# nianticlabs/panoptic-forecasting

Hardware: AMD Instinct MI355X
Metric: forecast frames/sec @1024x2048, 3-in->dt=3 bg (higher is better)
Workload: dtype f32 as 2 fp16 terms/operand, 3 MFMA products, f32 accumulate (strict f32: fp32_only); 1 GPU; configs[1] bg short-term forecast 3-in dt=3 @1024x2048: 3 warp/splats + HarDNet-70 + upsample/argmax; resident_frames_per_gpu=128, streams=4, sub_batch=32, launch=hipGraph replay, sub-batches staggered, weights=random-init, calibrated (tests/golden/calib_seed1234.json), world=1, device=AMD Radeon Graphics, backend=single process

## Files before the change

panoptic-forecasting_amd/csrc/conv_dma.hip:

```cpp
#include <cstring>

#include "conv_epilogue.h"
#include "pf_prof.h"

#ifndef PF_PROBE
#define PF_PROBE 0
#endif
#if PF_PROBE
#define DPROBE(i) do { if (threadIdx.x == 0 && blockIdx.x == 5 && blockIdx.y == 0 && blockIdx.z == 0 && a.probe) a.probe[i] = wall_clock64(); } while (0)
#else
#define DPROBE(i) do { } while (0)
#endif

namespace pf {

typedef float f32x4 __attribute__((ext_vector_type(4)));

template <int KS, int STRIDE, int WM, int WK, int NT, int RV = 0>
struct DmaCfg {
    static constexpr int KC = dma_kc_ct(KS, STRIDE);
    static constexpr int MP = 4;
    static constexpr int TWT = WM == 1 ? 1 : 2;
    static constexpr int TW = 16 * TWT;
    static constexpr int TH = WM * MP / TWT;
// ... 306 lines not shown
            const int ox = tileX * C::TW + (mt % C::TWT) * 16 + (lane_e >> 4) * 4;
            if (oy >= a.Hout || ox >= a.Wout) continue;
            const bool pool_top = a.pool && ((m / C::TWT) & 1) == 0 && m + C::TWT < C::MP && oy + 1 < a.Hout;
            if (a.pool && !pool_top) continue;
            ResTaps t0, t1;
            if (has_res) {
                t0 = res_taps(a, rw, oy, ox);
                if (pool_top) t1 = res_taps(a, rw, oy + 1, ox);
            }
#pragma unroll
            for (int n = 0; n < NT; ++n) {
                const int co = (tile0 + n) * 16 + (lane_e & 15);
                if (epi_skip(a, co)) continue;
                const lds_float *chan = res_lds + (n * 16 + (lane_e & 15)) * rw.cs;
                const f32x4 top = epi_finish(a, b, co, oy, ox, acc[m][n], biasv[n], has_res, chan, &t0);
                if (!a.pool) epi_store(a, b, co, oy, ox, top, vmax);
                else epi_store_pooled(a, b, co, oy, ox, top, epi_finish(a, b, co, oy + 1, ox, acc[(m + C::TWT) % C::MP][n], biasv[n], has_res, chan, &t1), vmax);
                __builtin_amdgcn_sched_barrier(0);
            }
            DPROBE(5 + m);
        }
    }
    range_commit(a.status, a.range_slot, vmax);
    DPROBE(4);
#endif
}

template <int KS, int STRIDE, int WM, int WK, int NT, int EPI, int RV = 0, int KACC = 0>
static int launch_dma_epi(const ConvArgs &a0, int B, hipStream_t s) {
    if constexpr (KACC == 0 && EPI == 0 && RV == 0 && KS == 3) {
        if (a0.kacc) return launch_dma_epi<KS, STRIDE, WM, WK, NT, EPI, RV, 1>(a0, B, s);
// ... 126 lines not shown
```

panoptic-forecasting_amd/csrc/conv_epilogue.h:

```cpp
#pragma once
#include "conv_mfma.h"

namespace pf {

typedef float epi_f32x4 __attribute__((ext_vector_type(4)));
typedef float epi_f32x2 __attribute__((ext_vector_type(2)));
typedef __attribute__((address_space(3))) float lds_float;

__device__ __forceinline__ void lin_coord(int o, float scale, int in_size, int &i0, int &i1, float &l0, float &l1) {
#pragma clang fp contract(off)
    const float r = scale * (float)o;
    i0 = min((int)r, in_size - 1);
    i1 = i0 + (i0 < in_size - 1 ? 1 : 0);
    l1 = fminf(fmaxf(r - (float)i0, 0.f), 1.f);
    l0 = 1.f - l1;
}


__host__ __device__ inline int res_extent(int n_out, float scale) { return (int)(scale * (float)(n_out - 1)) + 3; }
__host__ __device__ inline int res_chan_stride(int rows, int cols) { return (rows * cols) | 1; }

struct ResWin {
    int sy0, sx0, rows, cols, cs;
};

__device__ __forceinline__ ResWin res_window(const ConvArgs &a, int oy0, int th, int ox0, int tw) {
    ResWin w;
    const int oy1 = min(oy0 + th, a.Hout) - 1, ox1 = min(ox0 + tw, a.Wout) - 1;
    w.sy0 = min((int)(a.res_sh * (float)oy0), a.Hres - 1);
    w.sx0 = min((int)(a.res_sw * (float)ox0), a.Wres - 1);
    w.rows = min((int)(a.res_sh * (float)oy1), a.Hres - 1) + 2 - w.sy0;
    w.cols = min((int)(a.res_sw * (float)ox1), a.Wres - 1) + 2 - w.sx0;
    w.cs = res_chan_stride(w.rows, w.cols);
    return w;
}

__device__ __forceinline__ void res_stage(const ConvArgs &a, const ResWin &w, int b, int co0, int nco, lds_float *lds,
                                          int tid, int nthr) {
    const int per = w.rows * w.cols;
    const size_t plane = (size_t)a.Hres * a.Wres;
    const float *base = a.res + ((size_t)b * a.res_ctotal + a.res_choff + co0) * plane;
    for (int e0 = 0; e0 < per; e0 += 64) {
        const int e = e0 + (tid & 63);
        const int r = e / w.cols, x = e - r * w.cols;
        const size_t off = (size_t)min(w.sy0 + r, a.Hres - 1) * a.Wres + min(w.sx0 + x, a.Wres - 1);
#pragma unroll 4
        for (int c = tid >> 6; c < nco; c += nthr >> 6)
            if (e < per && co0 + c < a.Cout) lds[c * w.cs + e] = base[(size_t)c * plane + off];
    }
}

struct ResTaps {
    int o0[4], o1[4];
    float lx1[4], hy1;
};
__device__ __forceinline__ ResTaps res_taps(const ConvArgs &a, const ResWin &w, int oy, int ox) {
    ResTaps t;
    int y0, y1;
    float hy0;
    lin_coord(oy, a.res_sh, a.Hres, y0, y1, hy0, t.hy1);
#pragma unroll
    for (int r = 0; r < 4; ++r) {
        int x0, x1;
// ... 95 lines not shown
            *reinterpret_cast<epi_h2 *>(p + 4) = epi_h2{hi[0], hi[1]};
            *reinterpret_cast<epi_h2 *>(p + 4 + d.term) = epi_h2{mid[0], mid[1]};
        }
        if (ok1) {
            *reinterpret_cast<epi_h2 *>(p + d.hw * 8) = epi_h2{hi[2], hi[3]};
            *reinterpret_cast<epi_h2 *>(p + d.hw * 8 + d.term) = epi_h2{mid[2], mid[3]};
        }
    }
}
__device__ __forceinline__ epi_f32x4 s4_finish(epi_f32x4 acc, float scale, const epi_f32x4 &bias4, float relu_lo) {
#pragma unroll
    for (int r = 0; r < 4; ++r) acc[r] = fmaxf(acc[r] * scale + bias4[r], relu_lo);
    return acc;
}

__device__ __forceinline__ void epi_store(const ConvArgs &a, int b, int co, int oy, int ox, epi_f32x4 v, float &vmax) {
    vmax = range_acc(vmax, v[0], v[1], v[2], v[3]);
    if (a.dst_fmt) {
        if (co >= a.Cout) v = epi_f32x4{0.f, 0.f, 0.f, 0.f};
        const epi_f32x4 c = quad_transpose(v);
        const int k = threadIdx.x & 3;
        if (ox + k < a.Wout)
            s4_store_px(s4_dst(a, b, (size_t)a.Hout * a.Wout), co & ~3, (size_t)oy * a.Wout + ox + k, c);
        return;
    }
    float *p = a.dst + ((size_t)b * a.dst_ctotal + a.dst_choff + co) * ((size_t)a.Hout * a.Wout) + (size_t)oy * a.Wout + ox;
    if ((a.Wout & 3) == 0 && ox + 3 < a.Wout) {
        if (a.accum) v += *reinterpret_cast<const epi_f32x4 *>(p);
        *reinterpret_cast<epi_f32x4 *>(p) = v;
    } else {
#pragma unroll
        for (int r = 0; r < 4; ++r)
            if (ox + r < a.Wout) p[r] = a.accum ? p[r] + v[r] : v[r];
    }
}

__device__ __forceinline__ void epi_store_pooled(const ConvArgs &a, int b, int co, int oy, int ox, epi_f32x4 top, epi_f32x4 bot, float &vmax) {
    const int Hp = a.Hout >> 1, Wp = a.Wout >> 1, py = oy >> 1, px = ox >> 1;
// ... 23 lines not shown
```

panoptic-forecasting_amd/csrc/conv_mfma.h:

```cpp
#pragma once
#include "conv_pack.h"
#include "pf_blob.h"
#include "pf_common.h"

namespace pf {

struct ConvArgs {
    const float *src[kConvMaxSrc];
    int src_ctotal[kConvMaxSrc];
    int src_choff[kConvMaxSrc];
    int src_cstart[kConvMaxSrc + 1];
    int src_chunk0[kConvMaxSrc + 1];
    int n_src;
    const float *wpk;
    const float *bias;
    float *dst;
    int dst_ctotal, dst_choff;
    int Cin, Cout, Hin, Win, Hout, Wout;
    int tilesX, tilesY, nchunks, relu;
    const float *zero_page;
    int ntiles;
    int no_bias;
    int pool;
    const float *res;
    int res_ctotal, res_choff, Hres, Wres;
    float res_sh, res_sw;
    int res_lds_off;
    int res_rows, res_cols;
    unsigned res_magic_cs, res_magic_cols;
    const float *wrem;
    int rem;
    int src_begin, src_end;
    int chunk_begin, chunk_end;
    long long *probe;
    unsigned *status;
    unsigned *range_slot;
    int kacc;
    int accum;
    float acc_scale;
    int dst_fmt;
    int dst_c4;
    int dst_limit;
    int src_fmt;
    int src_c4[kConvMaxSrc];
    int src_g0[kConvMaxSrc];
    int src_gn[kConvMaxSrc];
    int src_ent0[kConvMaxSrc + 1];
    float *share;
    int share_off;
    int share_cout;
    float share_scale;
    const float *fold_w;
    const float *fold_bias;
    float fold_scale;
    const float *fold_src;
    int fold_c4, fold_g0, fold_gn;
    float *tail_dst;
    int fold_cout, tail_ctotal, tail_choff;
    float *down_dst;
    int down_c4, down_choff, down_limit;
    int down_fmt, down_ctotal;
    unsigned *down_status, *down_slot;
};

typedef _Float16 split_t;
typedef split_t split_x2 __attribute__((ext_vector_type(2)));
typedef split_t split_x4 __attribute__((ext_vector_type(4)));
typedef split_t split_x8 __attribute__((ext_vector_type(8)));
constexpr float kSplitMaxAbs = 65504.f;
__device__ __forceinline__ void split_terms2(float x0, float x1, split_x2 &hi, split_x2 &mid) {
#if defined(__HIP_DEVICE_COMPILE__)
    typedef float f32x2 __attribute__((ext_vector_type(2)));
    hi = __builtin_convertvector(f32x2{x0, x1}, split_x2);
// ... 220 lines not shown
```

panoptic-forecasting_amd/csrc/conv_s4.hip:

```cpp
#include <cstring>

#include "conv_s4.h"
#include "pf_prof.h"

#ifndef PF_PROBE
#define PF_PROBE 0
#endif
#if PF_PROBE
#define S4_PROBE(i) do { if (threadIdx.x == 0 && blockIdx.x == gridDim.x / 2 && blockIdx.y == 0 && blockIdx.z == gridDim.z / 2 && a.probe && (i) < 60) a.probe[i] = clock64(); } while (0)
#else
#define S4_PROBE(i) do { } while (0)
#endif

[[maybe_unused]] constexpr int kS4IssueFirst = 1, kS4IssueStep = 2;

namespace pf {

template <int NT, int TW_, int TH_ = 8, int KS_ = 1>
struct S4Cfg {
    static constexpr int TW = TW_, TH = TH_, MTR = TW / 16, MP = 2 * MTR;
    static constexpr int KS = KS_;
    static constexpr int NW = TH / 2, NTHR = 64 * NW;
    static constexpr int IW = TW + 4, IH = TH + 2;
    static constexpr int ROWP = IW / 2, PIECES = IH * ROWP;
// ... 126 lines not shown
    if (a.share_cout != a.Cout) return fail(PF_EINVAL, "conv_s4 add: stored sums of %d channels for %d", a.share_cout, a.Cout);
    PF_S4_SHARE(S4_ADD)
}
#undef PF_S4_SHARE
static int check_fold(const ConvArgs &a, const char *who, int max_cout, int ntiles = 2) {
    if (int rc = check_s4_form(a, who, false)) return rc;
    if (a.ntiles != ntiles) return fail(PF_EUNSUPPORTED, "%s: %d cout tiles, the form is built for %d", who, a.ntiles, ntiles);
    if (!a.fold_w || !a.fold_bias || a.fold_cout < 1 || a.fold_cout > max_cout || a.fold_gn < 0 || a.fold_gn > 8 || (a.fold_gn && !a.fold_src) ||
        (reinterpret_cast<uintptr_t>(a.fold_w) & 15) != 0 || (reinterpret_cast<uintptr_t>(a.fold_bias) & 15) != 0 || a.fold_g0 < 0 ||
        a.fold_g0 + a.fold_gn > a.fold_c4)
        return fail(PF_EINVAL, "%s: second conv of %d couts over %d groups", who, a.fold_cout, a.fold_gn);
    return PF_OK;
}
int launch_conv_s4_tail(const ConvArgs &a, int B, hipStream_t s) {
    if (int rc = check_fold(a, "conv_s4 tail", 16)) return rc;
    if (!a.tail_dst || a.tail_choff < 0 || a.tail_choff + a.fold_cout > a.tail_ctotal)
        return fail(PF_EINVAL, "conv_s4 tail: second conv of %d couts over %d groups", a.fold_cout, a.fold_gn);
    return launch_s4_form<S4_TAIL, 2>(a, B, s);
}
int launch_conv_s4_down(const ConvArgs &a, int B, hipStream_t s) {
    const bool wide = a.ntiles == 3;
    if (int rc = check_fold(a, "conv_s4 down", 16 * (wide ? kWideTiles : kDownTiles), wide ? 3 : 2)) return rc;
    if (a.Hout < 2 || a.Wout < 2) return fail(PF_EUNSUPPORTED, "conv_s4 down: nothing to pool at %d x %d", a.Hout, a.Wout);
    const bool packed_ok = (a.down_choff & 1) == 0 && a.down_limit >= a.down_choff + a.fold_cout && a.down_limit <= 4 * a.down_c4 &&
                           a.down_limit <= (a.down_choff + a.fold_cout + 3) / 4 * 4;
    if (!a.down_dst || a.down_choff < 0 || (a.down_fmt ? !packed_ok : a.down_choff + a.fold_cout > a.down_ctotal))
        return fail(PF_EINVAL, "conv_s4 down: pooled destination of %d channels from %d (limit %d) in %d groups", a.fold_cout, a.down_choff, a.down_limit, a.down_c4);
    return wide ? launch_s4_form<S4_DOWN, 3>(a, B, s) : launch_s4_form<S4_DOWN, 2>(a, B, s);
}
int launch_conv_s4_lo(const ConvArgs &a, int B, hipStream_t s) {
    if (int rc = check_fold(a, "conv_s4 lo", 16 * kLoTiles, 3)) return rc;
    if (!a.tail_dst || a.tail_choff < 0 || a.tail_choff + a.fold_cout > a.tail_ctotal)
        return fail(PF_EINVAL, "conv_s4 lo: second conv of %d couts over %d groups", a.fold_cout, a.fold_gn);
    return launch_s4_form<S4_LO, 3>(a, B, s);
}

int launch_conv_s4(const ConvArgs &a, int ks, const S4Shape &sh, int B, hipStream_t s) {
    if (!a.src_fmt) return fail(PF_EINVAL, "conv_s4: sources are not in the S4 layout");
    if ((a.Wout & 3) != 0 || a.Hin != a.Hout || a.Win != a.Wout) return fail(PF_EUNSUPPORTED, "conv_s4: stride 1, width % 4 == 0 only");
    if (ks == 3) {
        if (a.pool || a.res || a.no_bias) return fail(PF_EUNSUPPORTED, "conv_s4 3x3: no fused epilogue stages");
        if (a.chunk_begin != 0 || a.chunk_end != a.nchunks) return fail(PF_EUNSUPPORTED, "conv_s4 3x3: whole K range only");
#define PF_S4(FORM_, NT_, TW_, TH_, KS_) \
    if (sh.NT == NT_ && sh.TW == TW_ && sh.TH == TH_ && sh.KS == KS_) return launch_s4_form<FORM_, NT_, TW_, TH_, KS_>(a, B, s);
        if (a.kacc) {
            PF_S4(S4_BLOCKED, 1, 32, 8, 1) PF_S4(S4_BLOCKED, 2, 32, 8, 1) PF_S4(S4_BLOCKED, 3, 32, 8, 1)
        } else {
// ... 20 lines not shown
```

panoptic-forecasting_amd/csrc/conv_s4_1x1.hip:

```cpp
#include <cstring>

#include "conv_s4.h"
#include "pf_prof.h"

namespace pf {

template <int NT>
struct S41Cfg {
    static constexpr int TW = 32, TH = 8, MP = 4;
    static constexpr int WBUF = NT * 2 * 64 * 16;
    static constexpr int BIAS_OFF = 2 * WBUF;
    static constexpr int MAIN = 2 * WBUF + 256;
    static constexpr int WPIECES = WBUF / 16, NITW = (WPIECES + 255) / 256;
};

typedef unsigned s4_u32x4 __attribute__((ext_vector_type(4)));
typedef unsigned s4_u32x2 __attribute__((ext_vector_type(2)));

template <int NT, int EPI>
__global__ __launch_bounds__(256, NT <= 2 ? 4 : (NT == 3 ? 3 : 2)) void conv_s4_1x1_kernel(ConvArgs a) {
#if defined(__HIP_DEVICE_COMPILE__)
    using C = S41Cfg<NT>;
    extern __shared__ __attribute__((aligned(16))) unsigned char smem_raw[];
    const int tid = threadIdx.x, lane = tid & 63;
// ... 58 lines not shown
        for (int it = 0; it < C::NITW; ++it)
            if (it * 256 + tid < C::WPIECES)
                __builtin_amdgcn_raw_ptr_buffer_load_lds(wrsrc, (s4_lds_ptr_t)(wdst + (it * 256 + wave * 64) * 16), 16, woff[it],
                                                         (unsigned)(cb + r) * (2 * 64 * 16), 0, 0);
    };

    s4_u32x4 cur[2][2][2], nxt[2][2][2];
    if (nrounds > 0) {
        load_weights(0, wbuf(0));
        load_round(0, cur);
    }
    if (has_res) {
        rw = res_window(a, tileY * C::TH, C::TH, tileX * C::TW, C::TW);
        rw.rows = a.res_rows;
        rw.cols = a.res_cols;
        rw.cs = res_chan_stride(a.res_rows, a.res_cols);
        const unsigned per = (unsigned)(rw.rows * rw.cols), total = (unsigned)(NT * 16 * rw.cs);
        const size_t rplane = (size_t)a.Hres * a.Wres;
        const __amdgpu_buffer_rsrc_t rrs = __builtin_amdgcn_make_buffer_rsrc(
            (void *)(a.res + ((size_t)b * a.res_ctotal + a.res_choff + tile0 * 16) * rplane), 0, 0x7FFFFFFF, 0x00020000);
        unsigned char *rdst = smem_raw + a.res_lds_off * 4;
        for (unsigned e0 = (unsigned)wave * 64; e0 < total; e0 += 256) {
            const unsigned e = e0 + lane;
            const unsigned c = __umulhi(e, a.res_magic_cs), rem = e - c * (unsigned)rw.cs;
            const unsigned r = __umulhi(rem, a.res_magic_cols), x = rem - r * (unsigned)rw.cols;
            const int row = min(rw.sy0 + (int)r, a.Hres - 1), col = min(rw.sx0 + (int)x, a.Wres - 1);
            const bool ok = e < total && rem < per && tile0 * 16 + (int)c < a.Cout;
            const unsigned off = ok ? (unsigned)((c * rplane + (size_t)row * a.Wres + col) * 4) : kS4Oob;
            __builtin_amdgcn_raw_ptr_buffer_load_lds(rrs, (s4_lds_ptr_t)(rdst + e0 * 4), 4, off, 0, 0, 0);
        }
    }

    for (int round = 0; round < nrounds; ++round) {
        asm volatile("s_waitcnt vmcnt(0)" ::: "memory");
        __syncthreads();
        const bool more = round + 1 < nrounds;
        if (more) {
            load_weights(round + 1, wbuf((round + 1) & 1));
            load_round(round + 1, nxt);
        }
        const unsigned char *wb = wbuf(round & 1);
        s4_h8 bh[NT], bm[NT];
#pragma unroll
        for (int n = 0; n < NT; ++n) {
// ... 20 lines not shown
#pragma unroll
            for (int rr = 0; rr < 2; ++rr)
#pragma unroll
                for (int h = 0; h < 2; ++h)
#pragma unroll
                    for (int t = 0; t < 2; ++t) cur[rr][h][t] = nxt[rr][h][t];
        }
    }

    if (has_res) {
        asm volatile("s_waitcnt vmcnt(0)" ::: "memory");
        __syncthreads();
    }
    {
        __builtin_amdgcn_s_waitcnt(0x0F70);
        const lds_float *res_lds = (const lds_float *)(reinterpret_cast<float *>(smem_raw) + (has_res ? a.res_lds_off : 0));
        const int i2 = 2 * (lane & 15);
        const int ox = tileX * C::TW + i2;
        const bool pooled = EPI == 1 && a.pool;
        const int Ho = pooled ? a.Hout >> 1 : a.Hout, Wo = pooled ? a.Wout >> 1 : a.Wout;
        const size_t hw = (size_t)Ho * Wo;
        const S4Dst sd = s4_dst(a, b, hw);
        float vmax = 0.f;
        const float relu_lo1 = a.relu ? 0.f : -__builtin_inff();
        auto finish = [&](int rr, int q, int n, const int (&o0)[2], const int (&o1)[2], const float (&lx1)[2], float hy1) {
            s4_f32x4 v = acc[rr * 2 + q][n];
            const s4_f32x4 b4 = *reinterpret_cast<const s4_f32x4 *>(bias_lds + n * 16 + 4 * g);
#pragma unroll
            for (int r = 0; r < 4; ++r) {
                v[r] = v[r] * a.acc_scale + b4[r];
                if (has_res) {
                    const lds_float *chan = res_lds + (n * 16 + 4 * g + r) * rw.cs;
                    const float lx0 = 1.f - lx1[q], hy0 = 1.f - hy1;
                    const float t0 = lx0 * chan[o0[q]] + lx1[q] * chan[o0[q] + 1];
                    const float t1 = lx0 * chan[o1[q]] + lx1[q] * chan[o1[q] + 1];
                    v[r] += hy0 * t0 + hy1 * t1;
                }
                v[r] = fmaxf(v[r], relu_lo1);
            }
            vmax = range_acc(vmax, v[0], v[1], v[2], v[3]);
            return v;
        };
        auto store_px = [&](int co, size_t pix, s4_f32x4 v) {
            if (a.dst_fmt) {
                s4_store_px(sd, co, pix, v);
            } else {
#pragma unroll
                for (int r = 0; r < 4; ++r)
                    if (co + r < a.Cout) a.dst[((size_t)b * a.dst_ctotal + a.dst_choff + co + r) * hw + pix] = v[r];
            }
        };
        auto store_pair = [&](int co, size_t pix, s4_f32x4 v0, s4_f32x4 v1) {
            const int chb = a.dst_choff + co;
            if (a.dst_fmt && (sd.choff & 2) == 0 && chb + 2 < sd.limit) {
                s4_h4 h0, m0, h1, m1;
                split_terms4(v0, h0, m0);
                split_terms4(v1, h1, m1);
                const s4_h8 hi = s4_join(h0, h1), mid = s4_join(m0, m1);
                char *p = sd.base + pix * 8 + (size_t)(chb >> 2) * sd.hw * 8;
                *reinterpret_cast<s4_h8 *>(p) = hi;
                *reinterpret_cast<s4_h8 *>(p + sd.term) = mid;
            } else if (!a.dst_fmt) {
                typedef float f2 __attribute__((ext_vector_type(2)));
#pragma unroll
                for (int r = 0; r < 4; ++r)
                    if (co + r < a.Cout)
                        *reinterpret_cast<f2 *>(a.dst + ((size_t)b * a.dst_ctotal + a.dst_choff + co + r) * hw + pix) = f2{v0[r], v1[r]};
            } else {
                store_px(co, pix, v0);
                store_px(co, pix + 1, v1);
            }
        };
#pragma unroll
        for (int rr = 0; rr < 2; ++rr) {
            if (pooled && rr == 1) continue;
            const int oy = tileY * C::TH + 2 * wave + rr;
// ... 39 lines not shown
    }
#endif
}

template <int NT, int EPI>
int launch_s41_cfg(const ConvArgs &a0, int B, hipStream_t s) {
    using C = S41Cfg<NT>;
    ConvArgs a = a0;
    a.tilesX = (a.Wout + C::TW - 1) / C::TW;
    a.tilesY = (a.Hout + C::TH - 1) / C::TH;
    size_t lds = C::MAIN;
    a.res_lds_off = -1;
    if (a.res) {
        a.res_rows = res_extent(C::TH, a.res_sh);
        a.res_cols = res_extent(C::TW, a.res_sw);
        const int cs = res_chan_stride(a.res_rows, a.res_cols);
        const size_t need = (size_t)NT * 16 * cs * sizeof(float);
        if (need > 64 * 1024 || (size_t)NT * 16 * cs >= 65536) return fail(PF_EUNSUPPORTED, "conv_s4 1x1: residual window of %zu B does not fit LDS", need);
        a.res_magic_cs = (unsigned)(0x100000000ull / (unsigned)cs) + 1u;
        a.res_magic_cols = (unsigned)(0x100000000ull / (unsigned)a.res_cols) + 1u;
        a.res_lds_off = C::MAIN / 4;
        lds = C::MAIN + align_up(need, 256);
    }
    static size_t attr_lds = 0;
    if (lds > attr_lds) {
        PF_HIP_CHECK(hipFuncSetAttribute(reinterpret_cast<const void *>(&conv_s4_1x1_kernel<NT, EPI>),
                                         hipFuncAttributeMaxDynamicSharedMemorySize, (int)lds));
        attr_lds = lds;
    }
    char label[112];
    snprintf(label, sizeof(label), "void pf::conv_s4_1x1_kernel<%d, %d>(pf::ConvArgs)", NT, EPI);
    if (a.res) strncat(label, " +res", sizeof(label) - strlen(label) - 1);
    if (a.pool) strncat(label, " +pool", sizeof(label) - strlen(label) - 1);
    if (a.no_bias) strncat(label, " lowres-half", sizeof(label) - strlen(label) - 1);
    const double px = (double)B * a.Hout * a.Wout;
    ProfScope ps(s, label, 2.0 * px * a.Cout * a.Cin, 4.0 * ((double)B * a.Cin * a.Hin * a.Win + px * a.Cout + (double)a.Cout * a.Cin));
    hipLaunchKernelGGL((conv_s4_1x1_kernel<NT, EPI>), dim3(a.tilesX * a.tilesY, (a.ntiles + NT - 1) / NT, B), dim3(256), lds, s, a);
// ... 12 lines not shown
```

panoptic-forecasting_amd/csrc/conv_s4_kernel.inc:

```
template <int NT, int TW_, int TH_, int KS_>
__global__ __launch_bounds__(32 * TH_ * KS_, S4_KERNEL_WAVES) void S4_KERNEL_NAME(ConvArgs a) {
    [[maybe_unused]] constexpr int KACC = S4_KERNEL_KACC;
    [[maybe_unused]] constexpr int EPI = S4_KERNEL_EPI;
#if defined(__HIP_DEVICE_COMPILE__)
    using C = S4Cfg<NT, TW_, TH_, KS_>;
    extern __shared__ __attribute__((aligned(16))) unsigned char smem_all[];
    const int lane = threadIdx.x & 63;
    const int wave_all = __builtin_amdgcn_readfirstlane((int)threadIdx.x >> 6);
    const int kgrp = C::KS > 1 ? wave_all / C::NW : 0;
    const int wave = C::KS > 1 ? wave_all % C::NW : wave_all;
    const int tid = C::KS > 1 ? (int)threadIdx.x & (C::NTHR - 1) : (int)threadIdx.x;
    unsigned char *const smem_raw = smem_all + kgrp * C::STAGES_BYTES;
    int tid_lin, cgroup;
    xcd_tile_order(a.tilesX * a.tilesY, tid_lin, cgroup);
    const int tileY = tid_lin / a.tilesX, tileX = tid_lin - tileY * a.tilesX;
    const int tile0 = cgroup * NT, b = blockIdx.z;
    const int iy0 = tileY * C::TH - 1, ix0 = tileX * C::TW - 2;
    const size_t plane_bytes = (size_t)a.Hin * a.Win * 8;
    auto abuf = [&](int i) { return smem_raw + i * C::ABUF; };
    auto wbuf = [&](int i) { return smem_raw + 2 * C::ABUF + i * C::WBUF; };

    s4_f32x4 acc[C::MP][NT];
    [[maybe_unused]] s4_f32x4 tot[KACC ? C::MP : 1][KACC ? NT : 1];
#pragma unroll
// ... 469 lines not shown
            const float *rbias = reinterpret_cast<const float *>(smem_all + FRAG_BYTES);
#pragma unroll 1
            for (int ct = 0; ct < rt; ++ct) {
                const s4_h8 wh0 = *reinterpret_cast<const s4_h8 *>(fw + (ct * 6 + 0) * 1024), wm0 = *reinterpret_cast<const s4_h8 *>(fw + (ct * 6 + 1) * 1024);
                const s4_h8 wh1 = *reinterpret_cast<const s4_h8 *>(fw + (ct * 6 + 2) * 1024), wm1 = *reinterpret_cast<const s4_h8 *>(fw + (ct * 6 + 3) * 1024);
                const s4_h8 wh2 = *reinterpret_cast<const s4_h8 *>(fw + (ct * 6 + 4) * 1024), wm2 = *reinterpret_cast<const s4_h8 *>(fw + (ct * 6 + 5) * 1024);
                const s4_f32x4 b4 = *reinterpret_cast<const s4_f32x4 *>(rbias + ct * 16 + 4 * g);
                const int co = ct * 16 + 4 * g;
#pragma unroll
                for (int m = 0; m < C::MP; ++m) {
                    const int mt = wave * C::MP + m;
                    const int oy = tileY * C::TH + mt / C::MTR;
                    const int ox = tileX * C::TW + (mt % C::MTR) * 16 + px;
                    s4_f32x4 t = fold_products(wh0, wm0, wh1, wm1, dx0h[m], dx0m[m], dx1h[m], dx1m[m]);
                    t = fold_products2(t, wh2, wm2, dx2h[m], dx2m[m]);
                    if (oy < a.Hout && ox < a.Wout) {
                        const size_t pix = (size_t)oy * a.Wout + ox;
#pragma unroll
                        for (int r = 0; r < 4; ++r)
                            if (co + r < a.fold_cout)
                                a.tail_dst[((size_t)b * a.tail_ctotal + a.tail_choff + co + r) * hw + pix] = t[r] * a.fold_scale + b4[r];
                    }
                }
            }
        }
        range_commit(a.status, a.range_slot, vmax);
    }
    S4_PROBE(59);
#endif
}
```

panoptic-forecasting_amd/csrc/conv_split.hip:

```cpp
#include <cstring>

#include "conv_epilogue.h"
#include "pf_prof.h"

#ifndef PF_PROBE
#define PF_PROBE 0
#endif
#if PF_PROBE
#define SPLIT_PROBE(i) do { if (threadIdx.x == 0 && blockIdx.x == gridDim.x / 2 && blockIdx.y == 0 && blockIdx.z == gridDim.z / 2 && a.probe && (i) < 60) a.probe[i] = clock64(); } while (0)
#else
#define SPLIT_PROBE(i) do { } while (0)
#endif

namespace pf {

typedef float sp_f32x4 __attribute__((ext_vector_type(4)));
typedef split_x8 sp_h8;
typedef __attribute__((address_space(3))) void *sp_lds_ptr_t;
[[maybe_unused]] constexpr unsigned kSplitOob = 0x80000000u;

template <int NT, int TW_>
struct SplitCfg {
    static constexpr int KC = 8, TW = TW_, TH = 8, MTR = TW / 16, MP = 2 * MTR;
    static constexpr int IW = TW + 8, IH = TH + 2, NPIX = IH * IW;
// ... 416 lines not shown
            const int ox = tileX * C::TW + (mt % C::MTR) * 16 + (lane_e >> 4) * 4;
            if (oy >= a.Hout || ox >= a.Wout) continue;
            const bool pool_top = a.pool && ((m / C::MTR) & 1) == 0 && m + C::MTR < C::MP && oy + 1 < a.Hout;
            if (a.pool && !pool_top) continue;
            ResTaps t0, t1;
            if (has_res) {
                t0 = res_taps(a, rw, oy, ox);
                if (pool_top) t1 = res_taps(a, rw, oy + 1, ox);
            }
#pragma unroll
            for (int n = 0; n < NT; ++n) {
                const int co = (tile0 + n) * 16 + (lane_e & 15);
                if (epi_skip(a, co)) continue;
                const lds_float *chan = res_lds + (n * 16 + (lane_e & 15)) * rw.cs;
                const sp_f32x4 top = epi_finish(a, b, co, oy, ox, acc[m][n] * a.acc_scale, biasv[n], has_res, chan, &t0);
                if (!a.pool) epi_store(a, b, co, oy, ox, top, vmax);
                else epi_store_pooled(a, b, co, oy, ox, top, epi_finish(a, b, co, oy + 1, ox, acc[(m + C::MTR) % C::MP][n] * a.acc_scale, biasv[n], has_res, chan, &t1), vmax);
                __builtin_amdgcn_sched_barrier(0);
            }
        }
    }
    range_commit(a.status, a.range_slot, vmax);
#endif
}

bool conv_split1_supported(const ConvArgs &a, int nt) {
    nt = nt < 1 ? 1 : (nt > a.ntiles ? a.ntiles : nt);
    nt = nt > 4 ? 4 : nt;
    return (a.Wout & 3) == 0 && a.Hin == a.Hout && a.Win == a.Wout &&
           (!a.res || (size_t)nt * 16 * res_chan_stride(res_extent(8, a.res_sh), res_extent(32, a.res_sw)) * sizeof(float) <= 64 * 1024);
}
// ... 46 lines not shown
```

panoptic-forecasting_amd/csrc/conv_wave.hip:

```cpp
#include <cstring>

#include "conv_epilogue.h"
#include "pf_prof.h"

#ifndef PF_PROBE
#define PF_PROBE 0
#endif
#if PF_PROBE
#define PROBE() do { if (lane == 0 && blockIdx.x == 0 && blockIdx.y == 0 && wk == 0 && a.probe && np < 60) a.probe[np++] = clock64(); } while (0)
#else
#define PROBE() do { } while (0)
#endif

namespace pf {

typedef float f32x4 __attribute__((ext_vector_type(4)));
typedef float f32x2 __attribute__((ext_vector_type(2)));

template <int KS, int MH, int NT, int WK>
struct WaveCfg {
    static constexpr int KC = wave_kc_ct(KS);
    static constexpr int KG = KC / 4;
    static constexpr int KS2 = KS * KS;
    static constexpr int NV = KG * KS2;
// ... 223 lines not shown
                if (a.relu) v[r] = fmaxf(v[r], 0.f);
            }
            epi_store(a, b, co, oy, ox, v, vmax);
        } else {
            const lds_float *chan = res_lds + (n * 16 + (lane_e & 15)) * rw.cs;
            ResTaps t0, t1;
            if (has_res) {
                t0 = res_taps(a, rw, oy, ox);
                if (a.pool && oy + 1 < a.Hout) t1 = res_taps(a, rw, oy + 1, ox);
            }
            const f32x4 top = epi_finish(a, b, co, oy, ox, total(m), biasv[n], has_res, chan, &t0);
            if (a.pool) {
                if (MH > 1 && oy + 1 < a.Hout)
                    epi_store_pooled(a, b, co, oy, ox, top, epi_finish(a, b, co, oy + 1, ox, total(MH > 1 ? m + 1 : m), biasv[n], has_res, chan, &t1), vmax);
            } else {
                epi_store(a, b, co, oy, ox, top, vmax);
            }
            __builtin_amdgcn_sched_barrier(0);
        }
    }
    range_commit(a.status, a.range_slot, vmax);
#endif
}

template <int KS, int MH, int NT, int WK, int EPI>
static int launch_wave_epi(const ConvArgs &a0, int B, hipStream_t s) {
    using C = WaveCfg<KS, MH, NT, WK>;
    static_assert(wave_lds_bytes(KS, MH, NT, WK) == C::LDS_FLOATS * sizeof(float), "wave_lds_bytes (conv_mfma.h) mirrors WaveCfg");
    ConvArgs a = a0;
    a.tilesX = (a.Wout + 15) / 16;
    a.tilesY = (a.Hout + MH - 1) / MH;
// ... 55 lines not shown
```

panoptic-forecasting_amd/csrc/hardnet_schedule.cpp:

```cpp
#include <algorithm>
#include <cstring>

#include "hardnet_schedule.h"
#include "pf_prof.h"

namespace pf {

int layout(const pf_plan *p, int B, int H, int W, std::vector<Dims> &d, std::vector<size_t> &off, size_t &total, size_t *share_off) {
    int rc = propagate_dims(p->net, H, W, d);
    if (rc) return rc;
    off.assign(p->net.tensors.size(), (size_t)-1);
    size_t cur = kStatusBytes;
    const uint32_t input = p->net.ops[0].src[0].tensor;
    for (size_t t = 0; t < p->net.tensors.size(); ++t) {
        if (t == input || d[t].h == 0) continue;
        off[t] = cur;
        cur += align_up((size_t)B * ((p->net.tensors[t].channels + 3) / 4 * 4) * d[t].h * d[t].w * sizeof(float), 256);
    }
    size_t share_bytes = 0;
    const int Bt = p->opt.table_batch > 0 ? p->opt.table_batch : B;
    for (size_t i = 1; i < p->net.ops.size(); ++i) {
        const BlobOp &P = p->net.ops[i - 1], &C = p->net.ops[i];
        const Dims &o = d[C.dst];
        if (p->conv[i].share_a_off && p->opt.share_s && share_wanted((int)P.cin, (int)P.cout, (int)C.cin, (int)C.cout, o.h, o.w, Bt, p->opt.share_s))
// ... 119 lines not shown
    a.zero_page = p->dev_weights;
    a.ntiles = ((int)o.cout + 15) / 16;
    a.acc_scale = 1.0f;
    a.status = status_of(o.dst); a.range_slot = slot_of(ci, o.dst);
    return st;
}

void Sched::choose(Step &st, int need) {
    const BlobOp &o = p->net.ops[st.ci];
    const ConvPlan &cp = p->conv[st.ci];
    const ConvArgs &a = st.u.c;
    const bool generic = (a.Win & 3) != 0;
    st.dec = decide_conv({(int)o.k, (int)o.stride, a.Cin, a.Cout, a.Hout, a.Wout, Bt, need, generic, cp.split_off != 0, cp.s4_off != 0,
                          p->opt.use_tuned_table != 0, p->opt.split_f16 != 0, false, cp.s4_rounds, conv_force()});
    st.need = need; st.sb = a.src_begin; st.se = a.src_end;
    const bool res_fits = !a.res || (size_t)st.dec.s4.NT * 16 * res_chan_stride(res_extent(8, a.res_sh), res_extent(32, a.res_sw)) * sizeof(float) <= 60 * 1024;
    st.can_read = s4_allowed && o.kind == OP_CONV && st.dec.wants_s4 && res_fits && ((a.src_begin == 0 && a.src_end == a.n_src) || cp.s4_pad);
    st.can_write_s4 = s4_allowed && !generic && (a.dst_choff & 1) == 0;
    st.can_write = st.can_write_s4 && (st.dec.ch.is(CONV_DMA) || st.dec.ch.is(CONV_SPLIT));
    st.u.c.dst_limit = claim(st.dst_t, a.dst_choff, a.dst_choff + a.Cout);
}

int Sched::walk_ops() {
    cand[input] = 0;
    for (size_t i = 0; i < p->net.ops.size(); ++i) {
        const BlobOp &o = p->net.ops[i];
        const Dims in = d[o.src[0].tensor];
        const Dims out = o.kind == OP_HEAD ? in : d[o.dst];
        int rc = PF_OK;
        if (o.kind == OP_STEM && stem) rc = stem_op(i, out);
        else if (o.kind == OP_STEM || o.kind == OP_CONV) rc = conv_op(i, in, out);
// ... 77 lines not shown
        a.pool = 1; a.dst = tptr(pool->dst); a.dst_ctotal = (int)p->net.tensors[pool->dst].channels;
        st.dst_t = pool->dst;
        a.status = status_of(pool->dst); a.range_slot = slot_of(i, pool->dst);
        ++i;
    }
    choose(st, pool ? 2 : 0);
    return PF_OK;
}

bool Sched::can_commute_upsample(size_t i, const Dims &in, const Dims &out) const {
    if (!fuse || !fuse_up || i + 1 >= p->net.ops.size()) return false;
    const BlobOp &o = p->net.ops[i], &n = p->net.ops[i + 1];
    return n.kind == OP_CONV && n.k == 1 && n.stride == 1 && n.n_src == 2 && n.src[0].tensor == o.dst &&
           n.src[0].choff == 0 && n.src[0].ch == p->net.tensors[o.dst].channels && p->readers[o.dst] == 1 &&
           (in.w & 3) == 0 && (out.w & 3) == 0 && n.cout <= p->net.tensors[o.dst].channels &&
           2 * in.h <= out.h + 1 && 2 * in.w <= out.w + 1;
}

void Sched::commuted_upsample(size_t &i, const Dims &in, const Dims &out) {
    const BlobOp &o = p->net.ops[i], &n = p->net.ops[i + 1];
    const Dims hi = out;
    cand[o.dst] = 0;
    auto tag_half = [&](Step &st, const char *half, int cin, const Dims &dd) {
        if (tags)
            snprintf(st.tag, sizeof(st.tag), "%02zu%c %s.%s %d->%u %dx%d", i + 1, half[0] == 'l' ? 'a' : 'b', p->net.tensors[n.dst].name,
                     half, cin, n.cout, dd.h, dd.w);
    };
    const KOrder kn = order_plain(n.src, (int)n.n_src);
    KOrder kx = kn;
    kx.r[0].tensor = o.src[0].tensor; kx.r[0].choff = (int)o.src[0].choff;
    Step &ls = conv_step(i, i + 1, kx, in, in);
    ConvArgs &lo = ls.u.c;
    lo.dst = tptr(o.dst);
    ls.dst_t = o.dst;
    lo.dst_ctotal = (int)n.cout; lo.dst_choff = 0;
    lo.relu = 0; lo.no_bias = 1;
    lo.status = nullptr; lo.range_slot = nullptr;
    lo.Cin = (int)n.src[0].ch;
    lo.src_end = 1;
    tag_half(ls, "lo", lo.Cin, in);
    choose(ls, 4);
    Step &hs = conv_step(i, i + 1, kn, hi, hi);
    ConvArgs &ha = hs.u.c;
    ha.Cin = (int)n.src[1].ch;
    ha.src_begin = 1; ha.src_end = 2;
    tag_half(hs, "hi", ha.Cin, hi);
    ha.res = tptr(o.dst); ha.res_ctotal = (int)n.cout;
    ha.Hres = in.h; ha.Wres = in.w;
    ha.res_sh = hi.h > 1 ? (float)(in.h - 1) / (float)(hi.h - 1) : 0.f;
    ha.res_sw = hi.w > 1 ? (float)(in.w - 1) / (float)(hi.w - 1) : 0.f;
// ... 186 lines not shown
}

void Sched::fold(FoldForm form) {
    const FoldDesc &f = kFolds[form];
    const int mode = p->opt.*f.option;
    for (size_t k = 0; mode && p->fold[form].dev && k + 1 < steps.size(); ++k) {
        Step &sl = steps[k];
        const Step &sr = steps[k + 1];
        const size_t i = (size_t)sl.op;
        if (sl.kind != S_CONV_S4 || sr.kind != S_CONV_S4 || sl.ci != (int)i || sr.op != (int)i + 1 || sr.ci != (int)(i + f.r_at())) continue;
        if (!p->conv[i].fold_off[form] || !is_conv_fold(p->net, i, form)) continue;
        const BlobOp &L = p->net.ops[i], &R = p->net.ops[i + f.r_at()];
        const ConvArgs &a = sl.u.c, &r = sr.u.c;
        const S4Shape &sh = sl.dec.s4;
        if (sh.NT != f.l_tiles || sh.TW != 32 || sh.TH != 8 || sh.KS != 1 || !a.dst_fmt || r.res || a.Hout != r.Hout || a.Wout != r.Wout) continue;
        if (f.up ? (!r.no_bias || r.relu || r.src_begin != 0 || r.src_end != 1 || r.dst_fmt || r.status || r.pool)
                 : r.no_bias || (form == FOLD_TAIL ? (r.dst_fmt || r.status || r.pool) : (!r.pool || !r.relu)))
            continue;
        if (!f.wanted((int)L.cin, (int)L.cout, (int)R.cout, a.Hout, a.Wout, Bt, mode)) continue;
        fold_into(sl, sr, form);
        steps.erase(steps.begin() + (long)k + 1);
    }
}

void Sched::fold_into(Step &sl, const Step &sr, FoldForm form) {
    const FoldDesc &f = kFolds[form];
    const size_t i = (size_t)sl.op;
    const BlobOp &L = p->net.ops[i], &R = p->net.ops[i + f.r_at()];
    ConvArgs &a = sl.u.c;
    const ConvArgs &r = sr.u.c;
    const KOrder ko = order_tail(p->net.ops[i + 1].src[0], (int)L.dst_choff, (int)L.cout);
    a.fold_w = p->fold[form].dev + p->conv[i].fold_off[form];
    a.fold_bias = f.up ? a.zero_page : r.bias; a.fold_scale = r.acc_scale; a.fold_cout = r.Cout;
    a.fold_src = a.dst; a.fold_c4 = a.dst_c4; a.fold_g0 = ko.r[0].choff / 4; a.fold_gn = ko.r[0].ch / 4;
    if (form == FOLD_TAIL || form == FOLD_LO) {
        a.tail_dst = r.dst; a.tail_ctotal = r.dst_ctotal; a.tail_choff = r.dst_choff;
        sl.kind = form == FOLD_TAIL ? S_CONV_S4_TAIL : S_CONV_S4_LO;
        bool read_elsewhere = false;
        for (size_t j = 0; j < p->net.ops.size(); ++j)
            for (uint32_t q = 0; q < p->net.ops[j].n_src && j != i + 1; ++q) {
                const BlobSrc &os = p->net.ops[j].src[q];
                read_elsewhere = read_elsewhere || (os.tensor == L.dst && os.choff < L.dst_choff + L.cout && os.choff + os.ch > L.dst_choff);
            }
        if (form == FOLD_TAIL || !read_elsewhere) {
            fmt[L.dst] = 0xFE;
            if (form == FOLD_LO) a.dst = nullptr;
        }
    } else {
        a.down_dst = r.dst; a.down_c4 = r.dst_c4; a.down_choff = r.dst_choff; a.down_limit = r.dst_limit;
        a.down_fmt = r.dst_fmt; a.down_ctotal = r.dst_ctotal;
        a.down_status = r.status; a.down_slot = r.range_slot;
// ... 105 lines not shown
```

Baseline: 3042 frames/s.

## Store low-resolution residual tensors in 4-channel grouped layout for vector loads

Residual tensors written by the low half of split up-convs are stored channel-grouped (four channels interleaved per pixel) instead of planar NCHW. Producers (epilogue stores, fold tails) write float4 groups, and the 1x1 s4 consumer stages the residual window with 16-byte DMA loads and reads float4 taps from LDS. This cuts the number of residual gather loads and LDS reads per output. In exchange it adds padding channels, alignment constraints, and some per-element stores in the generic epilogue path.

```diff
diff --git a/panoptic-forecasting_amd/csrc/conv_dma.hip b/panoptic-forecasting_amd/csrc/conv_dma.hip
--- a/panoptic-forecasting_amd/csrc/conv_dma.hip
+++ b/panoptic-forecasting_amd/csrc/conv_dma.hip
@@ -344,7 +344,7 @@
                 if (epi_skip(a, co)) continue;
                 const lds_float *chan = res_lds + (n * 16 + (lane_e & 15)) * rw.cs;
                 const f32x4 top = epi_finish(a, b, co, oy, ox, acc[m][n], biasv[n], has_res, chan, &t0);
-                if (!a.pool) epi_store(a, b, co, oy, ox, top, vmax);
+                if (!a.pool) epi_store<true>(a, b, co, oy, ox, top, vmax);
                 else epi_store_pooled(a, b, co, oy, ox, top, epi_finish(a, b, co, oy + 1, ox, acc[(m + C::TWT) % C::MP][n], biasv[n], has_res, chan, &t1), vmax);
                 __builtin_amdgcn_sched_barrier(0);
             }
diff --git a/panoptic-forecasting_amd/csrc/conv_epilogue.h b/panoptic-forecasting_amd/csrc/conv_epilogue.h
--- a/panoptic-forecasting_amd/csrc/conv_epilogue.h
+++ b/panoptic-forecasting_amd/csrc/conv_epilogue.h
@@ -6,6 +6,7 @@
 typedef float epi_f32x4 __attribute__((ext_vector_type(4)));
 typedef float epi_f32x2 __attribute__((ext_vector_type(2)));
 typedef __attribute__((address_space(3))) float lds_float;
+typedef __attribute__((address_space(3))) epi_f32x4 lds_f32x4;
 
 __device__ __forceinline__ void lin_coord(int o, float scale, int in_size, int &i0, int &i1, float &l0, float &l1) {
 #pragma clang fp contract(off)
@@ -35,18 +36,23 @@
     return w;
 }
 
+__host__ __device__ inline size_t res_grp_index(int b, int c4, int c, size_t plane_px, size_t pix) {
+    return ((((size_t)b * c4 + (size_t)(c >> 2)) * plane_px + pix) << 2) + (size_t)(c & 3);
+}
+__host__ __device__ inline int res_groups(int channels) { return (channels + 3) >> 2; }
+
 __device__ __forceinline__ void res_stage(const ConvArgs &a, const ResWin &w, int b, int co0, int nco, lds_float *lds,
                                           int tid, int nthr) {
     const int per = w.rows * w.cols;
     const size_t plane = (size_t)a.Hres * a.Wres;
-    const float *base = a.res + ((size_t)b * a.res_ctotal + a.res_choff + co0) * plane;
+    const int c4 = res_groups(a.res_ctotal);
     for (int e0 = 0; e0 < per; e0 += 64) {
         const int e = e0 + (tid & 63);
         const int r = e / w.cols, x = e - r * w.cols;
         const size_t off = (size_t)min(w.sy0 + r, a.Hres - 1) * a.Wres + min(w.sx0 + x, a.Wres - 1);
 #pragma unroll 4
         for (int c = tid >> 6; c < nco; c += nthr >> 6)
-            if (e < per && co0 + c < a.Cout) lds[c * w.cs + e] = base[(size_t)c * plane + off];
+            if (e < per && co0 + c < a.Cout) lds[c * w.cs + e] = a.res[res_grp_index(b, c4, a.res_choff + co0 + c, plane, off)];
     }
 }
 
@@ -172,6 +178,7 @@
     return acc;
 }
 
+template <bool GRP = false>
 __device__ __forceinline__ void epi_store(const ConvArgs &a, int b, int co, int oy, int ox, epi_f32x4 v, float &vmax) {
     vmax = range_acc(vmax, v[0], v[1], v[2], v[3]);
     if (a.dst_fmt) {
@@ -180,6 +187,15 @@
         const int k = threadIdx.x & 3;
         if (ox + k < a.Wout)
             s4_store_px(s4_dst(a, b, (size_t)a.Hout * a.Wout), co & ~3, (size_t)oy * a.Wout + ox + k, c);
+        return;
+    }
+    if (GRP && a.dst_grp) {
+        const size_t hw = (size_t)a.Hout * a.Wout;
+        const int c4 = res_groups(a.dst_ctotal), cend = co == a.Cout - 1 ? ((co + 4) & ~3) : co + 1;
+#pragma unroll
+        for (int r = 0; r < 4; ++r)
+            for (int c = co; c < cend && ox + r < a.Wout; ++c)
+                a.dst[res_grp_index(b, c4, a.dst_choff + c, hw, (size_t)oy * a.Wout + ox + r)] = c == co ? v[r] : 0.f;
         return;
     }
     float *p = a.dst + ((size_t)b * a.dst_ctotal + a.dst_choff + co) * ((size_t)a.Hout * a.Wout) + (size_t)oy * a.Wout + ox;
diff --git a/panoptic-forecasting_amd/csrc/conv_mfma.h b/panoptic-forecasting_amd/csrc/conv_mfma.h
--- a/panoptic-forecasting_amd/csrc/conv_mfma.h
+++ b/panoptic-forecasting_amd/csrc/conv_mfma.h
@@ -27,7 +27,8 @@
     float res_sh, res_sw;
     int res_lds_off;
     int res_rows, res_cols;
-    unsigned res_magic_cs, res_magic_cols;
+    unsigned res_magic_per, res_magic_cols;
+    int dst_grp;
     const float *wrem;
     int rem;
     int src_begin, src_end;
@@ -57,6 +58,7 @@
     int fold_c4, fold_g0, fold_gn;
     float *tail_dst;
     int fold_cout, tail_ctotal, tail_choff;
+    int tail_grp;
     float *down_dst;
     int down_c4, down_choff, down_limit;
     int down_fmt, down_ctotal;
diff --git a/panoptic-forecasting_amd/csrc/conv_s4.hip b/panoptic-forecasting_amd/csrc/conv_s4.hip
--- a/panoptic-forecasting_amd/csrc/conv_s4.hip
+++ b/panoptic-forecasting_amd/csrc/conv_s4.hip
@@ -164,7 +164,7 @@
 }
 int launch_conv_s4_tail(const ConvArgs &a, int B, hipStream_t s) {
     if (int rc = check_fold(a, "conv_s4 tail", 16)) return rc;
-    if (!a.tail_dst || a.tail_choff < 0 || a.tail_choff + a.fold_cout > a.tail_ctotal)
+    if (!a.tail_dst || a.tail_grp || a.tail_choff < 0 || a.tail_choff + a.fold_cout > a.tail_ctotal)
         return fail(PF_EINVAL, "conv_s4 tail: second conv of %d couts over %d groups", a.fold_cout, a.fold_gn);
     return launch_s4_form<S4_TAIL, 2>(a, B, s);
 }
@@ -180,7 +180,8 @@
 }
 int launch_conv_s4_lo(const ConvArgs &a, int B, hipStream_t s) {
     if (int rc = check_fold(a, "conv_s4 lo", 16 * kLoTiles, 3)) return rc;
-    if (!a.tail_dst || a.tail_choff < 0 || a.tail_choff + a.fold_cout > a.tail_ctotal)
+    if (!a.tail_dst || !a.tail_grp || a.tail_choff < 0 || (a.tail_choff & 3) != 0 || a.tail_choff + a.fold_cout > a.tail_ctotal ||
+        (reinterpret_cast<uintptr_t>(a.tail_dst) & 15) != 0)
         return fail(PF_EINVAL, "conv_s4 lo: second conv of %d couts over %d groups", a.fold_cout, a.fold_gn);
     return launch_s4_form<S4_LO, 3>(a, B, s);
 }
diff --git a/panoptic-forecasting_amd/csrc/conv_s4_1x1.hip b/panoptic-forecasting_amd/csrc/conv_s4_1x1.hip
--- a/panoptic-forecasting_amd/csrc/conv_s4_1x1.hip
+++ b/panoptic-forecasting_amd/csrc/conv_s4_1x1.hip
@@ -96,20 +96,20 @@
         rw = res_window(a, tileY * C::TH, C::TH, tileX * C::TW, C::TW);
         rw.rows = a.res_rows;
         rw.cols = a.res_cols;
-        rw.cs = res_chan_stride(a.res_rows, a.res_cols);
-        const unsigned per = (unsigned)(rw.rows * rw.cols), total = (unsigned)(NT * 16 * rw.cs);
+        rw.cs = a.res_rows * a.res_cols;
+        const unsigned total = (unsigned)(NT * 4 * rw.cs);
         const size_t rplane = (size_t)a.Hres * a.Wres;
-        const __amdgpu_buffer_rsrc_t rrs = __builtin_amdgcn_make_buffer_rsrc(
-            (void *)(a.res + ((size_t)b * a.res_ctotal + a.res_choff + tile0 * 16) * rplane), 0, 0x7FFFFFFF, 0x00020000);
+        const int c4 = res_groups(a.res_ctotal), grp0 = (a.res_choff >> 2) + tile0 * 4;
+        const __amdgpu_buffer_rsrc_t rrs = __builtin_amdgcn_make_buffer_rsrc((void *)(a.res + res_grp_index(b, c4, grp0 * 4, rplane, 0)), 0, 0x7FFFFFFF, 0x00020000);
         unsigned char *rdst = smem_raw + a.res_lds_off * 4;
         for (unsigned e0 = (unsigned)wave * 64; e0 < total; e0 += 256) {
             const unsigned e = e0 + lane;
-            const unsigned c = __umulhi(e, a.res_magic_cs), rem = e - c * (unsigned)rw.cs;
+            const unsigned c = __umulhi(e, a.res_magic_per), rem = e - c * (unsigned)rw.cs;
             const unsigned r = __umulhi(rem, a.res_magic_cols), x = rem - r * (unsigned)rw.cols;
             const int row = min(rw.sy0 + (int)r, a.Hres - 1), col = min(rw.sx0 + (int)x, a.Wres - 1);
-            const bool ok = e < total && rem < per && tile0 * 16 + (int)c < a.Cout;
-            const unsigned off = ok ? (unsigned)((c * rplane + (size_t)row * a.Wres + col) * 4) : kS4Oob;
-            __builtin_amdgcn_raw_ptr_buffer_load_lds(rrs, (s4_lds_ptr_t)(rdst + e0 * 4), 4, off, 0, 0, 0);
+            const bool ok = e < total && grp0 + (int)c < c4;
+            const unsigned off = ok ? (unsigned)((c * rplane + (size_t)row * a.Wres + col) * 16) : kS4Oob;
+            __builtin_amdgcn_raw_ptr_buffer_load_lds(rrs, (s4_lds_ptr_t)(rdst + e0 * 16), 16, off, 0, 0, 0);
         }
     }
 
@@ -160,7 +160,7 @@
     }
     {
         __builtin_amdgcn_s_waitcnt(0x0F70);
-        const lds_float *res_lds = (const lds_float *)(reinterpret_cast<float *>(smem_raw) + (has_res ? a.res_lds_off : 0));
+        const lds_f32x4 *res_lds = (const lds_f32x4 *)(reinterpret_cast<float *>(smem_raw) + (has_res ? a.res_lds_off : 0));
         const int i2 = 2 * (lane & 15);
         const int ox = tileX * C::TW + i2;
         const bool pooled = EPI == 1 && a.pool;
@@ -170,16 +170,21 @@
         float vmax = 0.f;
         const float relu_lo1 = a.relu ? 0.f : -__builtin_inff();
         auto finish = [&](int rr, int q, int n, const int (&o0)[2], const int (&o1)[2], const float (&lx1)[2], float hy1) {
+#pragma clang fp contract(off)
             s4_f32x4 v = acc[rr * 2 + q][n];
             const s4_f32x4 b4 = *reinterpret_cast<const s4_f32x4 *>(bias_lds + n * 16 + 4 * g);
+            s4_f32x4 c00 = v, c01 = v, c10 = v, c11 = v;
+            if (has_res) {
+                const lds_f32x4 *grp = res_lds + (n * 4 + g) * rw.cs;
+                c00 = grp[o0[q]]; c01 = grp[o0[q] + 1]; c10 = grp[o1[q]]; c11 = grp[o1[q] + 1];
+            }
 #pragma unroll
             for (int r = 0; r < 4; ++r) {
-                v[r] = v[r] * a.acc_scale + b4[r];
+                v[r] = __builtin_fmaf(v[r], a.acc_scale, b4[r]);
                 if (has_res) {
-                    const lds_float *chan = res_lds + (n * 16 + 4 * g + r) * rw.cs;
                     const float lx0 = 1.f - lx1[q], hy0 = 1.f - hy1;
-                    const float t0 = lx0 * chan[o0[q]] + lx1[q] * chan[o0[q] + 1];
-                    const float t1 = lx0 * chan[o1[q]] + lx1[q] * chan[o1[q] + 1];
+                    const float t0 = __builtin_fmaf(lx0, c00[r], lx1[q] * c01[r]);
+                    const float t1 = __builtin_fmaf(lx0, c10[r], lx1[q] * c11[r]);
                     v[r] += hy0 * t0 + hy1 * t1;
                 }
                 v[r] = fmaxf(v[r], relu_lo1);
@@ -190,6 +195,10 @@
         auto store_px = [&](int co, size_t pix, s4_f32x4 v) {
             if (a.dst_fmt) {
                 s4_store_px(sd, co, pix, v);
+            } else if (EPI == 1 && a.dst_grp) {
+#pragma unroll
+                for (int r = 0; r < 4; ++r) v[r] = co + r < a.Cout ? v[r] : 0.f;
+                if (co < a.Cout) *reinterpret_cast<s4_f32x4 *>(a.dst + res_grp_index(b, a.dst_c4, a.dst_choff + co, hw, pix)) = v;
             } else {
 #pragma unroll
                 for (int r = 0; r < 4; ++r)
@@ -206,6 +215,14 @@
                 char *p = sd.base + pix * 8 + (size_t)(chb >> 2) * sd.hw * 8;
                 *reinterpret_cast<s4_h8 *>(p) = hi;
                 *reinterpret_cast<s4_h8 *>(p + sd.term) = mid;
+            } else if (EPI == 1 && a.dst_grp) {
+                const bool odd = (lane & 1) != 0;
+                s4_f32x4 got;
+#pragma unroll
+                for (int r = 0; r < 4; ++r)
+                    got[r] = __builtin_bit_cast(float, __builtin_amdgcn_update_dpp(0, __builtin_bit_cast(int, odd ? v0[r] : v1[r]), 0xB1, 0xF, 0xF, true));
+                store_px(co, odd ? pix - 1 : pix, odd ? got : v0);
+                store_px(co, odd ? pix + 1 : pix + 2, odd ? v1 : got);
             } else if (!a.dst_fmt) {
                 typedef float f2 __attribute__((ext_vector_type(2)));
 #pragma unroll
@@ -275,13 +292,15 @@
     if (a.res) {
         a.res_rows = res_extent(C::TH, a.res_sh);
         a.res_cols = res_extent(C::TW, a.res_sw);
-        const int cs = res_chan_stride(a.res_rows, a.res_cols);
-        const size_t need = (size_t)NT * 16 * cs * sizeof(float);
-        if (need > 64 * 1024 || (size_t)NT * 16 * cs >= 65536) return fail(PF_EUNSUPPORTED, "conv_s4 1x1: residual window of %zu B does not fit LDS", need);
-        a.res_magic_cs = (unsigned)(0x100000000ull / (unsigned)cs) + 1u;
+        const int per = a.res_rows * a.res_cols;
+        const size_t need = align_up((size_t)NT * 4 * per, 64) * 16;
+        if (need > 64 * 1024) return fail(PF_EUNSUPPORTED, "conv_s4 1x1: residual window of %zu B does not fit LDS", need);
+        if ((a.res_choff & 3) != 0 || (size_t)a.Hres * a.Wres >= ((size_t)1 << 22))
+            return fail(PF_EUNSUPPORTED, "conv_s4 1x1: residual slice at channel %d of %d x %d", a.res_choff, a.Hres, a.Wres);
+        a.res_magic_per = (unsigned)(0x100000000ull / (unsigned)per) + 1u;
         a.res_magic_cols = (unsigned)(0x100000000ull / (unsigned)a.res_cols) + 1u;
         a.res_lds_off = C::MAIN / 4;
-        lds = C::MAIN + align_up(need, 256);
+        lds = C::MAIN + need;
     }
     static size_t attr_lds = 0;
     if (lds > attr_lds) {
diff --git a/panoptic-forecasting_amd/csrc/conv_s4_kernel.inc b/panoptic-forecasting_amd/csrc/conv_s4_kernel.inc
--- a/panoptic-forecasting_amd/csrc/conv_s4_kernel.inc
+++ b/panoptic-forecasting_amd/csrc/conv_s4_kernel.inc
@@ -507,12 +507,11 @@
                     const int ox = tileX * C::TW + (mt % C::MTR) * 16 + px;
                     s4_f32x4 t = fold_products(wh0, wm0, wh1, wm1, dx0h[m], dx0m[m], dx1h[m], dx1m[m]);
                     t = fold_products2(t, wh2, wm2, dx2h[m], dx2m[m]);
-                    if (oy < a.Hout && ox < a.Wout) {
-                        const size_t pix = (size_t)oy * a.Wout + ox;
-#pragma unroll
-                        for (int r = 0; r < 4; ++r)
-                            if (co + r < a.fold_cout)
-                                a.tail_dst[((size_t)b * a.tail_ctotal + a.tail_choff + co + r) * hw + pix] = t[r] * a.fold_scale + b4[r];
+                    if (oy < a.Hout && ox < a.Wout && co < a.fold_cout) {
+                        s4_f32x4 u;
+#pragma unroll
+                        for (int r = 0; r < 4; ++r) u[r] = co + r < a.fold_cout ? t[r] * a.fold_scale + b4[r] : 0.f;
+                        *reinterpret_cast<s4_f32x4 *>(a.tail_dst + res_grp_index(b, res_groups(a.tail_ctotal), a.tail_choff + co, hw, (size_t)oy * a.Wout + ox)) = u;
                     }
                 }
             }
diff --git a/panoptic-forecasting_amd/csrc/conv_split.hip b/panoptic-forecasting_amd/csrc/conv_split.hip
--- a/panoptic-forecasting_amd/csrc/conv_split.hip
+++ b/panoptic-forecasting_amd/csrc/conv_split.hip
@@ -454,7 +454,7 @@
                 if (epi_skip(a, co)) continue;
                 const lds_float *chan = res_lds + (n * 16 + (lane_e & 15)) * rw.cs;
                 const sp_f32x4 top = epi_finish(a, b, co, oy, ox, acc[m][n] * a.acc_scale, biasv[n], has_res, chan, &t0);
-                if (!a.pool) epi_store(a, b, co, oy, ox, top, vmax);
+                if (!a.pool) epi_store<true>(a, b, co, oy, ox, top, vmax);
                 else epi_store_pooled(a, b, co, oy, ox, top, epi_finish(a, b, co, oy + 1, ox, acc[(m + C::MTR) % C::MP][n] * a.acc_scale, biasv[n], has_res, chan, &t1), vmax);
                 __builtin_amdgcn_sched_barrier(0);
             }
diff --git a/panoptic-forecasting_amd/csrc/conv_wave.hip b/panoptic-forecasting_amd/csrc/conv_wave.hip
--- a/panoptic-forecasting_amd/csrc/conv_wave.hip
+++ b/panoptic-forecasting_amd/csrc/conv_wave.hip
@@ -261,7 +261,7 @@
                 if (MH > 1 && oy + 1 < a.Hout)
                     epi_store_pooled(a, b, co, oy, ox, top, epi_finish(a, b, co, oy + 1, ox, total(MH > 1 ? m + 1 : m), biasv[n], has_res, chan, &t1), vmax);
             } else {
-                epi_store(a, b, co, oy, ox, top, vmax);
+                epi_store<true>(a, b, co, oy, ox, top, vmax);
             }
             __builtin_amdgcn_sched_barrier(0);
         }
diff --git a/panoptic-forecasting_amd/csrc/hardnet_schedule.cpp b/panoptic-forecasting_amd/csrc/hardnet_schedule.cpp
--- a/panoptic-forecasting_amd/csrc/hardnet_schedule.cpp
+++ b/panoptic-forecasting_amd/csrc/hardnet_schedule.cpp
@@ -157,7 +157,7 @@
     st.dec = decide_conv({(int)o.k, (int)o.stride, a.Cin, a.Cout, a.Hout, a.Wout, Bt, need, generic, cp.split_off != 0, cp.s4_off != 0,
                           p->opt.use_tuned_table != 0, p->opt.split_f16 != 0, false, cp.s4_rounds, conv_force()});
     st.need = need; st.sb = a.src_begin; st.se = a.src_end;
-    const bool res_fits = !a.res || (size_t)st.dec.s4.NT * 16 * res_chan_stride(res_extent(8, a.res_sh), res_extent(32, a.res_sw)) * sizeof(float) <= 60 * 1024;
+    const bool res_fits = !a.res || (size_t)st.dec.s4.NT * 16 * (res_extent(8, a.res_sh) * res_extent(32, a.res_sw) + 4) * sizeof(float) <= 60 * 1024;
     st.can_read = s4_allowed && o.kind == OP_CONV && st.dec.wants_s4 && res_fits && ((a.src_begin == 0 && a.src_end == a.n_src) || cp.s4_pad);
     st.can_write_s4 = s4_allowed && !generic && (a.dst_choff & 1) == 0;
     st.can_write = st.can_write_s4 && (st.dec.ch.is(CONV_DMA) || st.dec.ch.is(CONV_SPLIT));
@@ -265,6 +265,7 @@
     return n.kind == OP_CONV && n.k == 1 && n.stride == 1 && n.n_src == 2 && n.src[0].tensor == o.dst &&
            n.src[0].choff == 0 && n.src[0].ch == p->net.tensors[o.dst].channels && p->readers[o.dst] == 1 &&
            (in.w & 3) == 0 && (out.w & 3) == 0 && n.cout <= p->net.tensors[o.dst].channels &&
+           (size_t)res_groups((int)n.cout) * 4 * in.h * in.w <= (size_t)p->net.tensors[o.dst].channels * out.h * out.w &&
            2 * in.h <= out.h + 1 && 2 * in.w <= out.w + 1;
 }
 
@@ -284,7 +285,7 @@
     ConvArgs &lo = ls.u.c;
     lo.dst = tptr(o.dst);
     ls.dst_t = o.dst;
-    lo.dst_ctotal = (int)n.cout; lo.dst_choff = 0;
+    lo.dst_ctotal = (int)n.cout; lo.dst_choff = 0; lo.dst_grp = 1;
     lo.relu = 0; lo.no_bias = 1;
     lo.status = nullptr; lo.range_slot = nullptr;
     lo.Cin = (int)n.src[0].ch;
@@ -501,8 +502,8 @@
         const ConvArgs &a = sl.u.c, &r = sr.u.c;
         const S4Shape &sh = sl.dec.s4;
         if (sh.NT != f.l_tiles || sh.TW != 32 || sh.TH != 8 || sh.KS != 1 || !a.dst_fmt || r.res || a.Hout != r.Hout || a.Wout != r.Wout) continue;
-        if (f.up ? (!r.no_bias || r.relu || r.src_begin != 0 || r.src_end != 1 || r.dst_fmt || r.status || r.pool)
-                 : r.no_bias || (form == FOLD_TAIL ? (r.dst_fmt || r.status || r.pool) : (!r.pool || !r.relu)))
+        if (f.up ? (!r.no_bias || !r.dst_grp || r.relu || r.src_begin != 0 || r.src_end != 1 || r.dst_fmt || r.status || r.pool)
+                 : r.no_bias || r.dst_grp || (form == FOLD_TAIL ? (r.dst_fmt || r.status || r.pool) : (!r.pool || !r.relu)))
             continue;
         if (!f.wanted((int)L.cin, (int)L.cout, (int)R.cout, a.Hout, a.Wout, Bt, mode)) continue;
         fold_into(sl, sr, form);
@@ -521,7 +522,7 @@
     a.fold_bias = f.up ? a.zero_page : r.bias; a.fold_scale = r.acc_scale; a.fold_cout = r.Cout;
     a.fold_src = a.dst; a.fold_c4 = a.dst_c4; a.fold_g0 = ko.r[0].choff / 4; a.fold_gn = ko.r[0].ch / 4;
     if (form == FOLD_TAIL || form == FOLD_LO) {
-        a.tail_dst = r.dst; a.tail_ctotal = r.dst_ctotal; a.tail_choff = r.dst_choff;
+        a.tail_dst = r.dst; a.tail_ctotal = r.dst_ctotal; a.tail_choff = r.dst_choff; a.tail_grp = r.dst_grp;
         sl.kind = form == FOLD_TAIL ? S_CONV_S4_TAIL : S_CONV_S4_LO;
         bool read_elsewhere = false;
         for (size_t j = 0; j < p->net.ops.size(); ++j)
```

Result: no change. 3035 frames/s (-0.2%).
